# WGLab/ContextSV

Measured on AMD Instinct MI355X. Metric: long reads scanned/s (whole-genome step: scan + depth + cluster + merge + CN + split passes), synthetic 30x ONT WGS, higher is better.
Workload: dtype u32

## Files before the change

### contextsv_amd/csrc/kernels/scan.hip

```cpp
#include <type_traits>

#include "../common.hpp"
#include "../devutil.hpp"

namespace csv {

constexpr int SCAN_THREADS = 256;
constexpr int SCAN_WAVES = SCAN_THREADS / WAVE;
constexpr uint32_t SIG_BUF = 512;
constexpr int RING_D = 4;
constexpr int SCAN_OCC = 6;
constexpr int CHUNK_WORDS = 4 * WAVE;

struct Chunk {
    uint32_t w[4];
};

__device__ __forceinline__ void glds16(const uint32_t *gbase, uint32_t lane_byte_off, uint32_t lds_dst)
{
    unsigned keep;
    asm volatile("s_mov_b32 %0, m0\n\ts_mov_b32 m0, %3\n\ts_nop 0\n\tglobal_load_lds_dwordx4 %1, %2\n\ts_mov_b32 m0, %0"
                 : "=&s"(keep) : "v"(lane_byte_off), "s"(gbase), "s"(lds_dst) : "memory");
}
__device__ __forceinline__ uint32_t lds_addr(const void *p) { return (uint32_t)(uintptr_t)(__attribute__((address_space(3))) const void *)p; }

__device__ __forceinline__ void ring_issue(uint32_t *slot, const uint32_t *__restrict__ cigar, uint64_t base, int lane, uint64_t n_cigar, int vec_ok)
{
    const uint64_t idx = base + (uint64_t)lane * 4;
    if (vec_ok && base + CHUNK_WORDS <= n_cigar) {
        glds16(cigar + base, (uint32_t)lane * 16u, (uint32_t)__builtin_amdgcn_readfirstlane((int)lds_addr(slot)));
    } else {
#pragma unroll
        for (int k = 0; k < 4; k++) slot[lane * 4 + k] = (idx + k < n_cigar) ? cigar[idx + k] : (uint32_t)OP_P;
    }
}

__device__ __forceinline__ void ring_wait_steady()
{
    static_assert(RING_D >= 2 && RING_D <= 8, "add the immediate for RING_D - 1");
    if (RING_D == 8) asm volatile("s_waitcnt vmcnt(7)" ::: "memory");
    if (RING_D == 7) asm volatile("s_waitcnt vmcnt(6)" ::: "memory");
    if (RING_D == 6) asm volatile("s_waitcnt vmcnt(5)" ::: "memory");
    if (RING_D == 5) asm volatile("s_waitcnt vmcnt(4)" ::: "memory");
    if (RING_D == 4) asm volatile("s_waitcnt vmcnt(3)" ::: "memory");
    if (RING_D == 3) asm volatile("s_waitcnt vmcnt(2)" ::: "memory");
    if (RING_D == 2) asm volatile("s_waitcnt vmcnt(1)" ::: "memory");
}
__device__ __forceinline__ void ring_wait_all() { asm volatile("s_waitcnt vmcnt(0)" ::: "memory"); }

__device__ __forceinline__ uint64_t wave_lower_bound(const uint64_t *__restrict__ cigar_off, uint64_t n, uint64_t target, int lane)
{
    uint64_t lo = 0, hi = n;
    while (hi - lo > 0) {
        const uint64_t span = hi - lo;
        const uint64_t step = (span + 63) / 64;
        const uint64_t probe = lo + (uint64_t)lane * step;
        const bool ge = probe >= hi || cigar_off[probe] >= target;
        const uint64_t m = __ballot(ge);
        const int first_ge = m ? __ffsll((long long)m) - 1 : 64;
        const uint64_t new_hi = first_ge < 64 ? min(lo + (uint64_t)first_ge * step, hi) : hi;
        const uint64_t new_lo = first_ge > 0 ? lo + (uint64_t)(first_ge - 1) * step + 1 : lo;
        if (first_ge == 0) return lo;
        lo = new_lo; hi = new_hi;
        if (step == 1) return hi;
    }
    return lo;
}

__device__ __forceinline__ uint32_t bcast32(uint32_t v, uint32_t i) { return (uint32_t)__builtin_amdgcn_readlane((int)v, (int)i); }
__device__ __forceinline__ uint64_t bcast64(uint64_t v, uint32_t i)
{
    return ((uint64_t)bcast32((uint32_t)(v >> 32), i) << 32) | bcast32((uint32_t)v, i);
}
__global__ __launch_bounds__(SCAN_THREADS, SCAN_OCC) void cigar_scan_kernel(
    uint64_t n_reads, uint64_t n_cigar, const int32_t *__restrict__ pos, const uint16_t *__restrict__ flag,
    const uint8_t *__restrict__ mapq, const uint64_t *__restrict__ cigar_off, const uint32_t *__restrict__ cigar,
    int vec_ok, uint32_t depth_len, uint32_t start_limit, uint32_t min_oplen, uint32_t min_mapq, int emit,
    csv_sig *__restrict__ sig_out, uint64_t sig_cap, int32_t *__restrict__ ref_end, int32_t *__restrict__ q_start,
    int32_t *__restrict__ q_end, uint32_t *__restrict__ ckpt, ScanCounters *__restrict__ cnt,
    unsigned long long *__restrict__ tile_range, uint32_t n_tiles, uint32_t *__restrict__ bucket_hist, int hist_type_pos, int hist_shift,
    const uint64_t *__restrict__ split)
{
    __shared__ csv_sig buf[SIG_BUF];
    __shared__ alignas(16) uint32_t ring[SCAN_WAVES][RING_D][CHUNK_WORDS];
    __shared__ uint32_t buf_n, blk_n_del, blk_overflow;
    __shared__ unsigned long long blk_gbase;

    const int lane = lane_id();
    const int wave = (int)uniform32(threadIdx.x >> 6);
    if (threadIdx.x == 0) { buf_n = 0; blk_n_del = 0; blk_overflow = 0; }

    uint32_t my_n_del = 0, my_overflow = 0, my_bucket_max = 0;

    const uint64_t n_waves = (uint64_t)gridDim.x * SCAN_WAVES;
    const uint64_t wave_gid = (uint64_t)blockIdx.x * SCAN_WAVES + wave;
    const uint64_t share = (n_cigar + n_waves - 1) / n_waves;
    __shared__ uint64_t split_s[SCAN_WAVES + 1];
    __shared__ uint64_t split_w[SCAN_WAVES + 1];
    if (split) {
        if (threadIdx.x <= SCAN_WAVES) {
            const uint64_t g = (uint64_t)blockIdx.x * SCAN_WAVES + threadIdx.x;
            split_s[threadIdx.x] = split[2 * g]; split_w[threadIdx.x] = split[2 * g + 1];
        }
    } else {
        const uint64_t b = wave_lower_bound(cigar_off, n_reads, wave_gid * share, lane);
        if (lane == 0) split_s[wave] = b;
        if (wave == SCAN_WAVES - 1) {
            const uint64_t e = (wave_gid + 1 >= n_waves) ? n_reads : wave_lower_bound(cigar_off, n_reads, (wave_gid + 1) * share, lane);
            if (lane == 0) split_s[SCAN_WAVES] = e;
        }
    }
    __syncthreads();
    const uint64_t r_begin = uniform64(split_s[wave]);
    const uint64_t r_end = uniform64(split_s[wave + 1]);

    const uint64_t w_begin = split ? uniform64(split_w[wave]) : uniform64(r_begin < r_end ? cigar_off[r_begin] : 0);
    const uint64_t w_end = split ? uniform64(split_w[wave + 1]) : uniform64(r_begin < r_end ? cigar_off[r_end] : 0);
    const uint64_t ring_base = w_begin & ~(uint64_t)(CHUNK_WORDS - 1);
    const uint32_t ring_total = r_begin < r_end ? (uint32_t)((w_end - ring_base + CHUNK_WORDS - 1) / CHUNK_WORDS) : 0u;
    uint32_t ring_ready = 0;
    for (uint32_t a = 0; a < (uint32_t)(RING_D - 1) && a < ring_total; a++)
        ring_issue(ring[wave][a], cigar, ring_base + (uint64_t)a * CHUNK_WORDS, lane, n_cigar, vec_ok);

    for (uint64_t rb = r_begin; rb < r_end; rb += WAVE) {
    const uint64_t nb_reads = min((uint64_t)WAVE, r_end - rb);
    uint64_t l_c0 = 0; uint32_t l_p0 = 0, l_flmq = 0, l_uns = 0;
    if ((uint64_t)lane < nb_reads) {
        const uint64_t rr = rb + lane;
        l_c0 = cigar_off[rr];
        const int32_t p = pos[rr];
        l_p0 = (uint32_t)p; l_flmq = (uint32_t)flag[rr] | ((uint32_t)mapq[rr] << 16);
        l_uns = (rr > 0 && p < pos[rr - 1]) ? 1u : 0u;
    }
    const uint64_t batch_end_word = uniform64(cigar_off[rb + nb_reads]);
    if (__ballot(l_uns != 0) && lane == 0) cnt->unsorted = 1u;
    for (uint32_t ri = 0; ri < (uint32_t)nb_reads; ri++) {
        const uint64_t r = rb + ri;
        const bool have_next = ri + 1 < (uint32_t)nb_reads;
        const uint64_t c0 = bcast64(l_c0, ri);
        const uint64_t c1 = have_next ? bcast64(l_c0, ri + 1) : batch_end_word;
        const uint32_t p0 = bcast32(l_p0, ri);
        const uint32_t flmq = bcast32(l_flmq, ri);
        const uint32_t fl = flmq & 0xffffu, mq = flmq >> 16;
        const bool emit_ok = emit && !(fl & (F_SECONDARY | F_UNMAP | F_DUP | F_QCFAIL | F_SUPP)) && mq >= min_mapq;

        uint32_t ref_carry = 0;
        uint32_t acc_q = 0;
        uint32_t acc_skip = 0;
        bool had_skip = false;
        int32_t  qs = -1;

        const uint32_t n_words = (uint32_t)(c1 - c0);
        const uint32_t head = (uint32_t)c0 & (uint32_t)(CHUNK_WORDS - 1);
        const uint32_t n_chunks = n_words ? (head + n_words + CHUNK_WORDS - 1) / CHUNK_WORDS : 0u;
        const uint32_t j0 = (uint32_t)((c0 - head - ring_base) / CHUNK_WORDS);
        uint32_t *__restrict__ const ck_read = ckpt + ((c0 - head) >> CKPT_SHIFT);
        int32_t rel = lane * 4 - (int32_t)head;
        for (uint32_t t = 0; t < n_chunks; t++, rel += CHUNK_WORDS) {
            const uint32_t j = j0 + t;
            if (j == ring_ready) {
                const uint32_t ahead = j + (RING_D - 1);
                if (ahead < ring_total) {
                    ring_issue(ring[wave][ahead % RING_D], cigar, ring_base + (uint64_t)ahead * CHUNK_WORDS, lane, n_cigar, vec_ok);
                    ring_wait_steady();
                } else {
                    ring_wait_all();
                }
                ring_ready = j + 1;
            }
            Chunk cur;
            {
                const uint4 v = *reinterpret_cast<const uint4 *>(&ring[wave][j % RING_D][lane * 4]);
                cur.w[0] = v.x; cur.w[1] = v.y; cur.w[2] = v.z; cur.w[3] = v.w;
            }

            const bool edge = (t == 0 && head != 0) || (t + 1) * CHUNK_WORDS - head > n_words;
            if (edge) {
#pragma unroll
                for (int k = 0; k < 4; k++) if (!((uint32_t)(rel + k) < n_words)) cur.w[k] = (uint32_t)OP_P;
            }
            uint32_t len[4], op[4], rl[4], ql[4];
            uint32_t lane_ref = 0, lane_q = 0, trig = 0, qst = 0;
#pragma unroll
            for (int k = 0; k < 4; k++) {
                op[k] = cur.w[k] & 15u;
                len[k] = cur.w[k] >> 4;
                rl[k] = len[k] & (uint32_t)__builtin_amdgcn_sbfe((int)(REF_OPS | (REF_OPS << 16)), cur.w[k], 1u);
                ql[k] = len[k] & (uint32_t)__builtin_amdgcn_sbfe((int)(QRY_OPS | (QRY_OPS << 16)), cur.w[k], 1u);
                lane_ref += rl[k];
                lane_q += ql[k];
                trig |= rl[k] ^ ql[k];
            }
            const bool big = trig >= min_oplen;
            if (qs < 0) {
#pragma unroll
                for (int k = 0; k < 4; k++) qst |= (QST_OPS >> op[k]) & 1u;
            }
            const uint32_t incl_ref = wave_incl_sum_dpp(lane_ref);
            {
                static_assert(CKPT_WORDS == 64, "one checkpoint per DPP row of 16 lanes x 4 words");
                uint32_t *__restrict__ ck = ck_read + t * (CHUNK_WORDS / CKPT_WORDS);
                const bool inside = (edge || t == 0) ? (rel > 0 && (uint32_t)rel < n_words) : true;
                if ((lane & 15) == 0 && inside) ck[lane >> 4] = ref_carry + (incl_ref - lane_ref);
            }
            const bool any_big = emit_ok && __ballot(big) != 0;
            const bool need_q = (qs < 0) || any_big;
            if (need_q) {
                const uint32_t q_carry = t ? wave_total_dpp(acc_q) : 0u;
                const uint32_t incl_q = wave_incl_sum_dpp(lane_q);
                const uint32_t rp = p0 + ref_carry + (incl_ref - lane_ref);
                const uint32_t qp = q_carry + (incl_q - lane_q);

                if (qs < 0) {
                    const uint64_t m = __ballot(qst != 0);
                    if (m) {
                        bool found = false;
                        uint32_t q_at = 0, acc = qp;
#pragma unroll
                        for (int k = 0; k < 4; k++) {
                            if (!found && ((QST_OPS >> op[k]) & 1u)) { found = true; q_at = acc; }
                            acc += ql[k];
                        }
                        qs = (int32_t)bcast32(q_at, (uint32_t)(__ffsll((long long)m) - 1));
                    }
                }

                if (any_big) {
                    uint32_t cand = 0, skipped = 0, lane_skip = 0;
                    {
                        uint32_t rpk = rp;
#pragma unroll
                        for (int k = 0; k < 4; k++) {
                            if (len[k] >= min_oplen) {
                                if (op[k] == OP_I || op[k] == OP_D) cand |= 1u << k;
                                else if (op[k] == OP_S) {
                                    if ((uint32_t)(rpk + 1u) >= depth_len) { skipped |= 1u << k; lane_skip += len[k]; }
                                    else cand |= 1u << k;
                                }
                            }
                            rpk += rl[k];
                        }
                    }
                    uint32_t skip_before = had_skip ? wave_total_dpp(acc_skip) : 0u;
                    if (__ballot(skipped != 0)) {
                        skip_before += wave_incl_sum_dpp(lane_skip) - lane_skip;
                        acc_skip += lane_skip;
                        had_skip = true;
                    }
                    if (__ballot(cand != 0)) {
                        uint32_t rpk = rp, qpk = qp, skk = skip_before;
#pragma unroll
                        for (int k = 0; k < 4; k++) {
                            if ((cand >> k) & 1u) {
                                csv_sig sg;
                                sg.start = rpk + 1u;
                                sg.end = sg.start + len[k] - 1u;
                                sg.read = (uint32_t)r;
                                const uint32_t kind = (op[k] == OP_I) ? CSV_KIND_INS : (op[k] == OP_D ? CSV_KIND_DEL : CSV_KIND_CLIP);
                                sg.qpos_kind = ((qpk - skk) << 2) | kind;
                                const uint32_t slot = atomicAdd(&buf_n, 1u);
                                if (slot < SIG_BUF) buf[slot] = sg;
                                else {
                                    const unsigned long long g = atomicAdd(&cnt->n_sig, 1ull);
                                    if (g < sig_cap) sig_out[g] = sg;
                                    if (bucket_hist) my_bucket_max = max(my_bucket_max, atomicAdd(&bucket_hist[bk_bucket(sg, hist_type_pos, hist_shift)], 1u) + 1u);
                                }
                                my_n_del += (kind == CSV_KIND_DEL);
                                my_overflow |= (sg.start >= start_limit);
                            }
                            if ((skipped >> k) & 1u) skk += len[k];
                            rpk += rl[k];
                            qpk += ql[k];
                        }
                    }
                }
            }
            acc_q += lane_q;
            ref_carry += (uint32_t)__builtin_amdgcn_readlane((int)incl_ref, 63);
        }

        if (tile_range && ref_carry != 0 && !(fl & (F_UNMAP | F_SECONDARY | F_QCFAIL | F_DUP))) {
            const uint32_t first = p0 + 1u, last = first + ref_carry - 1u;
            const uint32_t t0 = first >> DEPTH_TILE_SHIFT;
            if (t0 < n_tiles && last >= first) {
                const uint32_t t1 = min(last >> DEPTH_TILE_SHIFT, n_tiles - 1u);
                for (uint32_t t = t0 + (uint32_t)lane; t <= t1; t += WAVE) {
                    atomicMax(&tile_range[2 * (uint64_t)t], ~(unsigned long long)r);
                    atomicMax(&tile_range[2 * (uint64_t)t + 1], (unsigned long long)r + 1ull);
                }
            }
        }

        const uint32_t q_total = wave_total_dpp(acc_q);
        if (lane == 0) {
            uint32_t rlen = (fl & F_UNMAP) ? 0u : ref_carry;
            if (rlen == 0) rlen = 1;
            ref_end[r] = (int32_t)(p0 + rlen);
            q_start[r] = qs < 0 ? 0 : qs;
            q_end[r] = (int32_t)q_total;
        }
    }
    }
    ring_wait_all();

    if (!emit) return;
    my_n_del = wave_sum(my_n_del);
    const bool wave_overflow = __ballot(my_overflow != 0) != 0;
    if (lane == 0) {
        if (my_n_del) atomicAdd(&blk_n_del, my_n_del);
        if (wave_overflow) atomicOr(&blk_overflow, 1u);
    }
    __syncthreads();
    const uint32_t nb = min(buf_n, SIG_BUF);
    if (threadIdx.x == 0) {
        blk_gbase = nb ? atomicAdd(&cnt->n_sig, (unsigned long long)nb) : 0ull;
        if (blk_n_del) atomicAdd(&cnt->n_del, (unsigned long long)blk_n_del);
        if (blk_overflow) cnt->max_start = 0xffffffffu;
    }
    __syncthreads();
    const unsigned long long g = blk_gbase;
    for (uint32_t i = threadIdx.x; i < nb; i += SCAN_THREADS) {
        const csv_sig sg = buf[i];
        if (g + i < sig_cap) sig_out[g + i] = sg;
        if (bucket_hist) my_bucket_max = max(my_bucket_max, atomicAdd(&bucket_hist[bk_bucket(sg, hist_type_pos, hist_shift)], 1u) + 1u);
    }
    if (bucket_hist) {
        my_bucket_max = wave_max(my_bucket_max);
        if (lane == 0 && my_bucket_max > BK_LOCAL_MAX) atomicMax(&cnt->max_len, my_bucket_max);
    }
}

constexpr int RS_THREADS = 256;
constexpr int RS_WAVES = RS_THREADS / WAVE;
constexpr int rs_occ(int gl) { return gl == 8 ? 5 : 7; }
constexpr uint32_t TR_SLOTS = 64;
constexpr uint32_t RS_MIN_READS = 32;

template <int GL, bool PADDED>
__global__ __launch_bounds__(RS_THREADS, rs_occ(GL)) void cigar_scan_rows_kernel(
    uint64_t n_reads, uint64_t n_cigar, const int32_t *__restrict__ pos, const uint16_t *__restrict__ flag,
    const uint8_t *__restrict__ mapq, const uint64_t *__restrict__ cigar_off, const uint32_t *__restrict__ cigar,
    uint32_t depth_len, uint32_t start_limit, uint32_t min_oplen, uint32_t min_mapq, int emit,
    csv_sig *__restrict__ sig_out, uint64_t sig_cap, int32_t *__restrict__ ref_end, int32_t *__restrict__ q_start,
    int32_t *__restrict__ q_end, uint32_t *__restrict__ ckpt, ScanCounters *__restrict__ cnt,
    unsigned long long *__restrict__ tile_range, uint32_t n_tiles, uint32_t *__restrict__ bucket_hist, int hist_type_pos, int hist_shift,
    const uint64_t *__restrict__ split)
{
    constexpr int WPL = WAVE / GL;
    constexpr int NG = WAVE / GL;
    __shared__ csv_sig buf[SIG_BUF];
    __shared__ alignas(16) uint4 meta[RS_WAVES][WAVE];
    __shared__ uint32_t tr_first[TR_SLOTS], tr_last[TR_SLOTS];
    __shared__ uint32_t buf_n, blk_n_del, blk_overflow, tr_base;
    __shared__ unsigned long long blk_gbase;
    __shared__ uint64_t split_s[RS_WAVES + 1];

    const int lane = lane_id();
    const int wave = (int)uniform32(threadIdx.x >> 6);
    const uint32_t sub = (uint32_t)lane & (uint32_t)(GL - 1);
    const uint32_t grp = (uint32_t)lane / (uint32_t)GL;
    const uint32_t upper = (lane & 8) ? 0xffffffffu : 0u;
    if (threadIdx.x == 0) { buf_n = 0; blk_n_del = 0; blk_overflow = 0; }
    if (threadIdx.x < TR_SLOTS) { tr_first[threadIdx.x] = 0; tr_last[threadIdx.x] = 0; }

    const uint64_t n_waves = (uint64_t)gridDim.x * RS_WAVES;
    const uint64_t wave_gid = (uint64_t)blockIdx.x * RS_WAVES + wave;
    const uint64_t share = (n_cigar + n_waves - 1) / n_waves;
    if (split) {
        if (threadIdx.x <= RS_WAVES) split_s[threadIdx.x] = split[2 * ((uint64_t)blockIdx.x * RS_WAVES + threadIdx.x)];
    } else {
        const uint64_t b = wave_lower_bound(cigar_off, n_reads, wave_gid * share, lane);
        if (lane == 0) split_s[wave] = b;
        if (wave == RS_WAVES - 1) {
            const uint64_t e = (wave_gid + 1 >= n_waves) ? n_reads : wave_lower_bound(cigar_off, n_reads, (wave_gid + 1) * share, lane);
            if (lane == 0) split_s[RS_WAVES] = e;
        }
    }
    __syncthreads();
    if (threadIdx.x == 0) {
        const uint64_t r0 = split_s[0];
        tr_base = (tile_range && r0 < n_reads) ? (((uint32_t)pos[r0] + 1u) >> DEPTH_TILE_SHIFT) : 0u;
    }
    __syncthreads();
    const uint64_t r_begin = uniform64(split_s[wave]);
    const uint64_t r_end = uniform64(split_s[wave + 1]);
    const uint32_t tbase = tr_base;

    uint32_t my_n_del = 0, my_overflow = 0, my_bucket_max = 0;

    auto loadw = [&](uint32_t g, uint32_t (&w)[WPL]) {
        if (PADDED) {
#pragma unroll
            for (int q = 0; q < WPL; q += 4) {
                const uint4 x = *reinterpret_cast<const uint4 *>(cigar + g + q);
                w[q] = x.x; w[q + 1] = x.y; w[q + 2] = x.z; w[q + 3] = x.w;
            }
        } else {
#pragma unroll
            for (int k = 0; k < WPL; k++) w[k] = ((uint64_t)g + k < n_cigar) ? cigar[g + k] : (uint32_t)OP_P;
        }
    };

    for (uint64_t rb = r_begin; rb < r_end; rb += WAVE) {
        const uint32_t nb = (uint32_t)min((uint64_t)WAVE, r_end - rb);
        uint32_t l_p0 = 0, l_fl = 0;
        {
            uint4 m = make_uint4(0u, 0u, 0u, 0u);
            uint32_t l_uns = 0;
            if ((uint32_t)lane < nb) {
                const uint64_t rr = rb + lane;
                const uint64_t c0 = cigar_off[rr], c1 = cigar_off[rr + 1];
                const int32_t p = pos[rr];
                m = make_uint4((uint32_t)c0, (uint32_t)(c1 - c0), (uint32_t)p, (uint32_t)flag[rr] | ((uint32_t)mapq[rr] << 16));
                l_p0 = m.z; l_fl = m.w & 0xffffu;
                l_uns = (rr > 0 && p < pos[rr - 1]) ? 1u : 0u;
            }
            if (__ballot(l_uns != 0) && lane == 0) cnt->unsorted = 1u;
            __builtin_amdgcn_fence(__ATOMIC_RELEASE, "wavefront");
            meta[wave][lane] = m;
            __builtin_amdgcn_fence(__ATOMIC_RELEASE, "wavefront");
            __builtin_amdgcn_wave_barrier();
            __builtin_amdgcn_fence(__ATOMIC_ACQUIRE, "wavefront");
        }
        uint32_t slot = grp;
        bool act = slot < nb;
        uint4 cm = meta[wave][act ? slot : 0u];
        uint32_t v = 0;
        uint32_t ref_carry = 0, q_carry = 0, skip_carry = 0;
        int32_t qs = -1;
        uint32_t w[WPL];
        loadw(act ? (cm.x & ~3u) + sub * WPL : 0u, w);
        while (__ballot(act)) {
            const uint32_t c0 = cm.x, nw = act ? cm.y : 0u, p0 = cm.z, fl = cm.w & 0xffffu, mq = cm.w >> 16;
            const uint32_t a = c0 & ~3u;
            const uint32_t n_win = max(1u, (c0 - a + nw + 63u) >> 6);
            const bool last = v + 1 >= n_win;
            const uint32_t nslot = last ? slot + NG : slot;
            const bool nact = act && nslot < nb;
            uint4 nm = cm;
            if (last) nm = meta[wave][nact ? nslot : 0u];
            const uint32_t nv = last ? 0u : v + 1u;
            uint32_t wn[WPL];
            loadw(nact ? (nm.x & ~3u) + nv * 64u + sub * WPL : 0u, wn);

            const uint32_t g = a + v * 64u + sub * WPL;
            const uint32_t t = g - c0;
            const bool emit_ok = emit && act && !(fl & (F_SECONDARY | F_UNMAP | F_DUP | F_QCFAIL | F_SUPP)) && mq >= min_mapq;
            uint32_t lane_ref = 0, lane_q = 0, trig = 0;
#pragma unroll
            for (int k = 0; k < WPL; k++) {
                if (!((uint32_t)(t + k) < nw)) w[k] = (uint32_t)OP_P;
                const uint32_t len = w[k] >> 4;
                const uint32_t rl = len & (uint32_t)__builtin_amdgcn_sbfe((int)(REF_OPS | (REF_OPS << 16)), w[k], 1u);
                const uint32_t ql = len & (uint32_t)__builtin_amdgcn_sbfe((int)(QRY_OPS | (QRY_OPS << 16)), w[k], 1u);
                lane_ref += rl; lane_q += ql;
                trig |= rl ^ ql;
            }
            const uint32_t incl_ref = grp_incl_sum<GL>(lane_ref, upper);
            const uint32_t incl_q = grp_incl_sum<GL>(lane_q, upper);
            const uint32_t tot_ref = grp_last<GL>(incl_ref), tot_q = grp_last<GL>(incl_q);
            const uint32_t ro = ref_carry + (incl_ref - lane_ref);
            const uint32_t qp = q_carry + (incl_q - lane_q);
            {
                if ((g & (uint32_t)(CKPT_WORDS - 1)) == 0 && t - 1u < nw - 1u && nw) ckpt[g >> CKPT_SHIFT] = ro;
                if (WPL == 8 && ((g + 4u) & (uint32_t)(CKPT_WORDS - 1)) == 0 && t + 3u < nw - 1u && nw) {
                    uint32_t x = ro;
#pragma unroll
                    for (int k = 0; k < 4; k++) x += (w[k] >> 4) & (uint32_t)__builtin_amdgcn_sbfe((int)(REF_OPS | (REF_OPS << 16)), w[k], 1u);
                    ckpt[(g + 4u) >> CKPT_SHIFT] = x;
                }
            }
            if (__ballot(qs < 0 && act)) {
                uint32_t q_at = 0xffffffffu, acc = qp;
                bool found = false;
#pragma unroll
                for (int k = 0; k < WPL; k++) {
                    const uint32_t op = w[k] & 15u;
                    if (!found && ((QST_OPS >> op) & 1u)) { found = true; q_at = acc; }
                    acc += (w[k] >> 4) & (uint32_t)__builtin_amdgcn_sbfe((int)(QRY_OPS | (QRY_OPS << 16)), w[k], 1u);
                }
                const uint32_t first = grp_min<GL>(q_at);
                if (qs < 0 && first != 0xffffffffu) qs = (int32_t)first;
            }
            uint32_t skip_tot = 0;
            if (__ballot(emit_ok && trig >= min_oplen)) {
                constexpr uint32_t ISD_OPS = (1u << OP_I) | (1u << OP_S) | (1u << OP_D);
                uint32_t cand = 0, skipped = 0;
                if (emit_ok) {
#pragma unroll
                    for (int k = 0; k < WPL; k++)
                        if ((w[k] >> 4) >= min_oplen && __builtin_amdgcn_sbfe((int)(ISD_OPS | (ISD_OPS << 16)), w[k], 1u)) cand |= 1u << k;
                }
                const bool may_skip = ((p0 | ref_carry | tot_ref) >= 0x20000000u) || (p0 + ref_carry + tot_ref + 1u >= depth_len);
                uint32_t skip_before = skip_carry;
                if (__ballot(cand != 0 && may_skip)) {
                    uint32_t lane_skip = 0, rpk = p0 + ro;
#pragma unroll
                    for (int k = 0; k < WPL; k++) {
                        const uint32_t len = w[k] >> 4, op = w[k] & 15u;
                        if (((cand >> k) & 1u) && op == OP_S && (uint32_t)(rpk + 1u) >= depth_len) { skipped |= 1u << k; lane_skip += len; }
                        rpk += len & (uint32_t)__builtin_amdgcn_sbfe((int)(REF_OPS | (REF_OPS << 16)), w[k], 1u);
                    }
                    cand &= ~skipped;
                    const uint32_t is = grp_incl_sum<GL>(lane_skip, upper);
                    skip_before += is - lane_skip;
                    skip_tot = grp_last<GL>(is);
                }
                if (cand) {
                    uint32_t rpk = p0 + ro, qpk = qp, skk = skip_before;
#pragma unroll
                    for (int k = 0; k < WPL; k++) {
                        const uint32_t len = w[k] >> 4, op = w[k] & 15u;
                        if ((cand >> k) & 1u) {
                            csv_sig sg;
                            sg.start = rpk + 1u;
                            sg.end = sg.start + len - 1u;
                            sg.read = (uint32_t)rb + slot;
                            const uint32_t kind = (op == OP_I) ? CSV_KIND_INS : (op == OP_D ? CSV_KIND_DEL : CSV_KIND_CLIP);
                            sg.qpos_kind = ((qpk - skk) << 2) | kind;
                            const uint32_t sl = atomicAdd(&buf_n, 1u);
                            if (sl < SIG_BUF) buf[sl] = sg;
                            else {
                                const unsigned long long gi = atomicAdd(&cnt->n_sig, 1ull);
                                if (gi < sig_cap) sig_out[gi] = sg;
                                if (bucket_hist) my_bucket_max = max(my_bucket_max, atomicAdd(&bucket_hist[bk_bucket(sg, hist_type_pos, hist_shift)], 1u) + 1u);
                            }
                            my_n_del += (kind == CSV_KIND_DEL);
                            my_overflow |= (sg.start >= start_limit);
                        }
                        if ((skipped >> k) & 1u) skk += len;
                        rpk += len & (uint32_t)__builtin_amdgcn_sbfe((int)(REF_OPS | (REF_OPS << 16)), w[k], 1u);
                        qpk += len & (uint32_t)__builtin_amdgcn_sbfe((int)(QRY_OPS | (QRY_OPS << 16)), w[k], 1u);
                    }
                }
            }
            const uint32_t ref_total = ref_carry + tot_ref, q_total = q_carry + tot_q;
            if (last && act && sub == 0) meta[wave][slot] = make_uint4(ref_total, (uint32_t)qs, q_total, 0u);
            if (last) { ref_carry = 0; q_carry = 0; skip_carry = 0; qs = -1; v = 0; slot = nslot; cm = nm; act = nact; }
            else { ref_carry = ref_total; q_carry = q_total; skip_carry += skip_tot; v = nv; }
#pragma unroll
            for (int k = 0; k < WPL; k++) w[k] = wn[k];
        }
        __builtin_amdgcn_fence(__ATOMIC_RELEASE, "wavefront");
        __builtin_amdgcn_wave_barrier();
        __builtin_amdgcn_fence(__ATOMIC_ACQUIRE, "wavefront");
        {
            const bool mine = (uint32_t)lane < nb;
            const uint4 res = meta[wave][lane];
            const uint64_t rr = rb + lane;
            if (mine) {
                uint32_t rlen = (l_fl & F_UNMAP) ? 0u : res.x;
                if (rlen == 0) rlen = 1;
                ref_end[rr] = (int32_t)(l_p0 + rlen);
                q_start[rr] = (int32_t)res.y < 0 ? 0 : (int32_t)res.y;
                q_end[rr] = (int32_t)res.z;
            }
            uint32_t t0 = 1, t1 = 0;
            if (mine && tile_range && res.x != 0 && !(l_fl & (F_UNMAP | F_SECONDARY | F_QCFAIL | F_DUP))) {
                const uint32_t first = l_p0 + 1u, lastp = first + res.x - 1u;
                if ((first >> DEPTH_TILE_SHIFT) < n_tiles && lastp >= first) { t0 = first >> DEPTH_TILE_SHIFT; t1 = min(lastp >> DEPTH_TILE_SHIFT, n_tiles - 1u); }
            }
            auto mark = [&](uint32_t tt, uint32_t rd) {
                const uint32_t sl = tt - tbase;
                if (sl < TR_SLOTS) {
                    atomicMax(&tr_first[sl], ~rd);
                    atomicMax(&tr_last[sl], rd + 1u);
                } else {
                    atomicMax(&tile_range[2 * (uint64_t)tt], ~(unsigned long long)rd);
                    atomicMax(&tile_range[2 * (uint64_t)tt + 1], (unsigned long long)rd + 1ull);
                }
            };
            const bool wide = t1 >= t0 && t1 - t0 >= 8u;
            if (t1 >= t0 && !wide) for (uint32_t tt = t0; tt <= t1; tt++) mark(tt, (uint32_t)rr);
            for (uint64_t mw = __ballot(wide); mw; mw &= mw - 1) {
                const uint32_t src = (uint32_t)__builtin_ctzll(mw);
                const uint32_t a0 = bcast32(t0, src), a1 = bcast32(t1, src), rd = (uint32_t)rb + src;
                for (uint32_t tt = a0 + (uint32_t)lane; tt <= a1; tt += WAVE) mark(tt, rd);
            }
        }
        __builtin_amdgcn_fence(__ATOMIC_RELEASE, "wavefront");
        __builtin_amdgcn_wave_barrier();
    }
// ... 363 lines not shown
```

Baseline: 321.0 million.

## Add a specialized steady-state CIGAR chunk loop with hand-scheduled DPP scan

Splits the per-read chunk loop into a head chunk, a steady-state middle loop and a generic tail. The middle loop always issues the direct-to-LDS DMA, skips edge masking and the ring-ready checks, and interleaves the query-length decode with DPP prefix-sum steps behind sched_barriers. The query-start search is also computed in the head chunk with ballots rather than a separate scan. The aim is to cut per-chunk control overhead and DPP latency stalls in the dominant scan loop, at the cost of more code, an m0 clobber that relies on the compiler, and a more fragile ring-index bookkeeping.

Result: no change. 322.3 million (median of 3 runs) (+0.4%).

```diff
diff --git a/contextsv_amd/csrc/kernels/scan.hip b/contextsv_amd/csrc/kernels/scan.hip
--- a/contextsv_amd/csrc/kernels/scan.hip
+++ b/contextsv_amd/csrc/kernels/scan.hip
@@ -22,6 +22,14 @@
     asm volatile("s_mov_b32 %0, m0\n\ts_mov_b32 m0, %3\n\ts_nop 0\n\tglobal_load_lds_dwordx4 %1, %2\n\ts_mov_b32 m0, %0"
                  : "=&s"(keep) : "v"(lane_byte_off), "s"(gbase), "s"(lds_dst) : "memory");
 }
+#pragma clang diagnostic push
+#pragma clang diagnostic ignored "-Winline-asm"
+__device__ __forceinline__ void glds16_m0(const uint32_t *gbase, uint32_t lane_byte_off, uint32_t lds_dst)
+{
+    asm volatile("s_mov_b32 m0, %2\n\ts_nop 0\n\tglobal_load_lds_dwordx4 %0, %1"
+                 : : "v"(lane_byte_off), "s"(gbase), "s"(lds_dst) : "memory", "m0");
+}
+#pragma clang diagnostic pop
 __device__ __forceinline__ uint32_t lds_addr(const void *p) { return (uint32_t)(uintptr_t)(__attribute__((address_space(3))) const void *)p; }
 
 __device__ __forceinline__ void ring_issue(uint32_t *slot, const uint32_t *__restrict__ cigar, uint64_t base, int lane, uint64_t n_cigar, int vec_ok)
@@ -121,6 +129,9 @@
     uint32_t ring_ready = 0;
     for (uint32_t a = 0; a < (uint32_t)(RING_D - 1) && a < ring_total; a++)
         ring_issue(ring[wave][a], cigar, ring_base + (uint64_t)a * CHUNK_WORDS, lane, n_cigar, vec_ok);
+    const uint32_t dma_chunks = vec_ok ? (uint32_t)min((uint64_t)ring_total, (n_cigar - ring_base) / CHUNK_WORDS) : 0u;
+    const uint32_t ring_lds = uniform32(lds_addr(&ring[wave][0][0]));
+    const uint32_t lane16 = (uint32_t)lane * 16u;
 
     for (uint64_t rb = r_begin; rb < r_end; rb += WAVE) {
     const uint64_t nb_reads = min((uint64_t)WAVE, r_end - rb);
@@ -155,8 +166,83 @@
         const uint32_t n_chunks = n_words ? (head + n_words + CHUNK_WORDS - 1) / CHUNK_WORDS : 0u;
         const uint32_t j0 = (uint32_t)((c0 - head - ring_base) / CHUNK_WORDS);
         uint32_t *__restrict__ const ck_read = ckpt + ((c0 - head) >> CKPT_SHIFT);
-        int32_t rel = lane * 4 - (int32_t)head;
-        for (uint32_t t = 0; t < n_chunks; t++, rel += CHUNK_WORDS) {
+
+        auto decode = [&](const Chunk &cur, uint32_t (&rl)[4], uint32_t (&ql)[4], uint32_t &lane_ref, uint32_t &lane_q, uint32_t &trig) __attribute__((always_inline)) {
+            lane_ref = 0; lane_q = 0; trig = 0;
+#pragma unroll
+            for (int k = 0; k < 4; k++) {
+                const uint32_t len = cur.w[k] >> 4;
+                rl[k] = len & (uint32_t)__builtin_amdgcn_sbfe((int)(REF_OPS | (REF_OPS << 16)), cur.w[k], 1u);
+                ql[k] = len & (uint32_t)__builtin_amdgcn_sbfe((int)(QRY_OPS | (QRY_OPS << 16)), cur.w[k], 1u);
+                lane_ref += rl[k];
+                lane_q += ql[k];
+                trig |= rl[k] ^ ql[k];
+            }
+        };
+
+        auto signatures = [&](const Chunk &cur, uint32_t rp, uint32_t qp) __attribute__((always_inline)) {
+            uint32_t op[4], len[4], rl[4], ql[4];
+#pragma unroll
+            for (int k = 0; k < 4; k++) {
+                uint32_t w = cur.w[k];
+                asm volatile("" : "+v"(w));
+                op[k] = w & 15u;
+                len[k] = w >> 4;
+                rl[k] = len[k] & (uint32_t)__builtin_amdgcn_sbfe((int)(REF_OPS | (REF_OPS << 16)), w, 1u);
+                ql[k] = len[k] & (uint32_t)__builtin_amdgcn_sbfe((int)(QRY_OPS | (QRY_OPS << 16)), w, 1u);
+            }
+            uint32_t cand = 0, skipped = 0, lane_skip = 0;
+            {
+                uint32_t rpk = rp;
+#pragma unroll
+                for (int k = 0; k < 4; k++) {
+                    if (len[k] >= min_oplen) {
+                        if (op[k] == OP_I || op[k] == OP_D) cand |= 1u << k;
+                        else if (op[k] == OP_S) {
+                            if ((uint32_t)(rpk + 1u) >= depth_len) { skipped |= 1u << k; lane_skip += len[k]; }
+                            else cand |= 1u << k;
+                        }
+                    }
+                    rpk += rl[k];
+                }
+            }
+            uint32_t skip_before = had_skip ? wave_total_dpp(acc_skip) : 0u;
+            if (__ballot(skipped != 0)) {
+                skip_before += wave_incl_sum_dpp(lane_skip) - lane_skip;
+                acc_skip += lane_skip;
+                had_skip = true;
+            }
+            if (__ballot(cand != 0)) {
+                uint32_t rpk = rp, qpk = qp, skk = skip_before;
+#pragma unroll
+                for (int k = 0; k < 4; k++) {
+                    if ((cand >> k) & 1u) {
+                        csv_sig sg;
+                        sg.start = rpk + 1u;
+                        sg.end = sg.start + len[k] - 1u;
+                        sg.read = (uint32_t)r;
+                        const uint32_t kind = (op[k] == OP_I) ? CSV_KIND_INS : (op[k] == OP_D ? CSV_KIND_DEL : CSV_KIND_CLIP);
+                        sg.qpos_kind = ((qpk - skk) << 2) | kind;
+                        const uint32_t slot = atomicAdd(&buf_n, 1u);
+                        if (slot < SIG_BUF) buf[slot] = sg;
+                        else {
+                            const unsigned long long g = atomicAdd(&cnt->n_sig, 1ull);
+                            if (g < sig_cap) sig_out[g] = sg;
+                            if (bucket_hist) my_bucket_max = max(my_bucket_max, atomicAdd(&bucket_hist[bk_bucket(sg, hist_type_pos, hist_shift)], 1u) + 1u);
+                        }
+                        my_n_del += (kind == CSV_KIND_DEL);
+                        my_overflow |= (sg.start >= start_limit);
+                    }
+                    if ((skipped >> k) & 1u) skk += len[k];
+                    rpk += rl[k];
+                    qpk += ql[k];
+                }
+            }
+        };
+
+        auto visit = [&](auto is_head, const uint32_t t) __attribute__((always_inline)) {
+            constexpr bool HEAD = decltype(is_head)::value;
+            const int32_t rel = lane * 4 + (int32_t)(t * CHUNK_WORDS) - (int32_t)head;
             const uint32_t j = j0 + t;
             if (j == ring_ready) {
                 const uint32_t ahead = j + (RING_D - 1);
@@ -174,110 +260,120 @@
                 cur.w[0] = v.x; cur.w[1] = v.y; cur.w[2] = v.z; cur.w[3] = v.w;
             }
 
-            const bool edge = (t == 0 && head != 0) || (t + 1) * CHUNK_WORDS - head > n_words;
+            const bool edge = (HEAD && head != 0) || (t + 1) * CHUNK_WORDS - head > n_words;
             if (edge) {
 #pragma unroll
                 for (int k = 0; k < 4; k++) if (!((uint32_t)(rel + k) < n_words)) cur.w[k] = (uint32_t)OP_P;
             }
-            uint32_t len[4], op[4], rl[4], ql[4];
-            uint32_t lane_ref = 0, lane_q = 0, trig = 0, qst = 0;
-#pragma unroll
-            for (int k = 0; k < 4; k++) {
-                op[k] = cur.w[k] & 15u;
-                len[k] = cur.w[k] >> 4;
-                rl[k] = len[k] & (uint32_t)__builtin_amdgcn_sbfe((int)(REF_OPS | (REF_OPS << 16)), cur.w[k], 1u);
-                ql[k] = len[k] & (uint32_t)__builtin_amdgcn_sbfe((int)(QRY_OPS | (QRY_OPS << 16)), cur.w[k], 1u);
-                lane_ref += rl[k];
-                lane_q += ql[k];
-                trig |= rl[k] ^ ql[k];
-            }
+            uint32_t rl[4], ql[4], lane_ref, lane_q, trig;
+            decode(cur, rl, ql, lane_ref, lane_q, trig);
             const bool big = trig >= min_oplen;
+            uint64_t qst_lanes = 0;
+            uint32_t pre_q = 0;
             if (qs < 0) {
-#pragma unroll
-                for (int k = 0; k < 4; k++) qst |= (QST_OPS >> op[k]) & 1u;
+                uint32_t h[4];
+#pragma unroll
+                for (int k = 0; k < 4; k++) h[k] = (uint32_t)__builtin_amdgcn_sbfe((int)(QST_OPS | (QST_OPS << 16)), cur.w[k], 1u);
+                uint32_t seen = h[0];
+                pre_q = ql[0] & ~seen;
+                seen |= h[1]; pre_q += ql[1] & ~seen;
+                seen |= h[2]; pre_q += ql[2] & ~seen;
+                seen |= h[3];
+                qst_lanes = __ballot(seen != 0);
+                if (HEAD && qst_lanes) {
+                    const uint32_t F = (uint32_t)__builtin_ctzll(qst_lanes);
+                    if ((__ballot(lane_q != 0) & ((1ull << F) - 1ull)) == 0) { qs = (int32_t)bcast32(pre_q, F); qst_lanes = 0; }
+                }
             }
             const uint32_t incl_ref = wave_incl_sum_dpp(lane_ref);
             {
                 static_assert(CKPT_WORDS == 64, "one checkpoint per DPP row of 16 lanes x 4 words");
                 uint32_t *__restrict__ ck = ck_read + t * (CHUNK_WORDS / CKPT_WORDS);
-                const bool inside = (edge || t == 0) ? (rel > 0 && (uint32_t)rel < n_words) : true;
+                const bool inside = (edge || HEAD) ? (rel > 0 && (uint32_t)rel < n_words) : true;
                 if ((lane & 15) == 0 && inside) ck[lane >> 4] = ref_carry + (incl_ref - lane_ref);
             }
             const bool any_big = emit_ok && __ballot(big) != 0;
-            const bool need_q = (qs < 0) || any_big;
-            if (need_q) {
-                const uint32_t q_carry = t ? wave_total_dpp(acc_q) : 0u;
+            if (qst_lanes != 0 || any_big) {
+                const uint32_t q_carry = HEAD ? 0u : wave_total_dpp(acc_q);
                 const uint32_t incl_q = wave_incl_sum_dpp(lane_q);
-                const uint32_t rp = p0 + ref_carry + (incl_ref - lane_ref);
                 const uint32_t qp = q_carry + (incl_q - lane_q);
-
-                if (qs < 0) {
-                    const uint64_t m = __ballot(qst != 0);
-                    if (m) {
-                        bool found = false;
-                        uint32_t q_at = 0, acc = qp;
-#pragma unroll
-                        for (int k = 0; k < 4; k++) {
-                            if (!found && ((QST_OPS >> op[k]) & 1u)) { found = true; q_at = acc; }
-                            acc += ql[k];
-                        }
-                        qs = (int32_t)bcast32(q_at, (uint32_t)(__ffsll((long long)m) - 1));
-                    }
-                }
-
-                if (any_big) {
-                    uint32_t cand = 0, skipped = 0, lane_skip = 0;
-                    {
-                        uint32_t rpk = rp;
-#pragma unroll
-                        for (int k = 0; k < 4; k++) {
-                            if (len[k] >= min_oplen) {
-                                if (op[k] == OP_I || op[k] == OP_D) cand |= 1u << k;
-                                else if (op[k] == OP_S) {
-                                    if ((uint32_t)(rpk + 1u) >= depth_len) { skipped |= 1u << k; lane_skip += len[k]; }
-                                    else cand |= 1u << k;
-                                }
-                            }
-                            rpk += rl[k];
-                        }
-                    }
-                    uint32_t skip_before = had_skip ? wave_total_dpp(acc_skip) : 0u;
-                    if (__ballot(skipped != 0)) {
-                        skip_before += wave_incl_sum_dpp(lane_skip) - lane_skip;
-                        acc_skip += lane_skip;
-                        had_skip = true;
-                    }
-                    if (__ballot(cand != 0)) {
-                        uint32_t rpk = rp, qpk = qp, skk = skip_before;
-#pragma unroll
-                        for (int k = 0; k < 4; k++) {
-                            if ((cand >> k) & 1u) {
-                                csv_sig sg;
-                                sg.start = rpk + 1u;
-                                sg.end = sg.start + len[k] - 1u;
-                                sg.read = (uint32_t)r;
-                                const uint32_t kind = (op[k] == OP_I) ? CSV_KIND_INS : (op[k] == OP_D ? CSV_KIND_DEL : CSV_KIND_CLIP);
-                                sg.qpos_kind = ((qpk - skk) << 2) | kind;
-                                const uint32_t slot = atomicAdd(&buf_n, 1u);
-                                if (slot < SIG_BUF) buf[slot] = sg;
-                                else {
-                                    const unsigned long long g = atomicAdd(&cnt->n_sig, 1ull);
-                                    if (g < sig_cap) sig_out[g] = sg;
-                                    if (bucket_hist) my_bucket_max = max(my_bucket_max, atomicAdd(&bucket_hist[bk_bucket(sg, hist_type_pos, hist_shift)], 1u) + 1u);
-                                }
-                                my_n_del += (kind == CSV_KIND_DEL);
-                                my_overflow |= (sg.start >= start_limit);
-                            }
-                            if ((skipped >> k) & 1u) skk += len[k];
-                            rpk += rl[k];
-                            qpk += ql[k];
-                        }
-                    }
-                }
+                if (qst_lanes) qs = (int32_t)bcast32(qp + pre_q, (uint32_t)__builtin_ctzll(qst_lanes));
+                if (any_big) signatures(cur, p0 + ref_carry + (incl_ref - lane_ref), qp);
             }
             acc_q += lane_q;
             ref_carry += (uint32_t)__builtin_amdgcn_readlane((int)incl_ref, 63);
-        }
+        };
+
+        uint32_t t = 0;
+        if (n_chunks) { visit(std::true_type{}, 0u); t = 1; }
+        if (qs >= 0 && n_chunks > 2) {
+            const uint32_t reach = j0 + (uint32_t)RING_D;
+            const uint32_t t_end = dma_chunks > reach ? min(n_chunks - 1u, dma_chunks - reach + 1u) : 1u;
+            if (t_end > 1u) {
+                uint32_t slot = ((j0 + (uint32_t)RING_D) % RING_D) * (uint32_t)(CHUNK_WORDS * 4);
+                const uint32_t *gp = cigar + ring_base + (uint64_t)reach * CHUNK_WORDS;
+                uint32_t *__restrict__ ck = ck_read + (CHUNK_WORDS / CKPT_WORDS) + (lane >> 4);
+                const bool ck_lane = (lane & 15) == 0;
+                for (; t < t_end; t++) {
+                    glds16_m0(gp, lane16, ring_lds + slot);
+                    ring_wait_steady();
+                    gp += CHUNK_WORDS;
+                    slot = (slot + (uint32_t)(CHUNK_WORDS * 4)) % (uint32_t)(RING_D * CHUNK_WORDS * 4);
+                    Chunk cur;
+                    {
+                        const uint4 v = *reinterpret_cast<const uint4 *>(reinterpret_cast<const char *>(&ring[wave][0][0]) + slot + lane16);
+                        cur.w[0] = v.x; cur.w[1] = v.y; cur.w[2] = v.z; cur.w[3] = v.w;
+                    }
+                    uint32_t rl[4], ql[4], lane_ref = 0, lane_q, trig = 0;
+                    const auto qlen = [&](int k) { return (cur.w[k] >> 4) & (uint32_t)__builtin_amdgcn_sbfe((int)(QRY_OPS | (QRY_OPS << 16)), cur.w[k], 1u); };
+#pragma unroll
+                    for (int k = 0; k < 4; k++) {
+                        rl[k] = (cur.w[k] >> 4) & (uint32_t)__builtin_amdgcn_sbfe((int)(REF_OPS | (REF_OPS << 16)), cur.w[k], 1u);
+                        lane_ref += rl[k];
+                    }
+                    uint32_t incl_ref = lane_ref;
+                    __builtin_amdgcn_sched_barrier(0);
+                    ql[0] = qlen(0); asm volatile("" : "+v"(ql[0]));
+                    __builtin_amdgcn_sched_barrier(0);
+                    incl_ref += dpp_u32<0x111, 0xf>(0u, incl_ref);
+                    __builtin_amdgcn_sched_barrier(0);
+                    ql[1] = qlen(1); asm volatile("" : "+v"(ql[1]));
+                    __builtin_amdgcn_sched_barrier(0);
+                    incl_ref += dpp_u32<0x112, 0xf>(0u, incl_ref);
+                    __builtin_amdgcn_sched_barrier(0);
+                    ql[2] = qlen(2); asm volatile("" : "+v"(ql[2]));
+                    __builtin_amdgcn_sched_barrier(0);
+                    incl_ref += dpp_u32<0x114, 0xf>(0u, incl_ref);
+                    __builtin_amdgcn_sched_barrier(0);
+                    ql[3] = qlen(3); asm volatile("" : "+v"(ql[3]));
+                    __builtin_amdgcn_sched_barrier(0);
+                    incl_ref += dpp_u32<0x118, 0xf>(0u, incl_ref);
+                    __builtin_amdgcn_sched_barrier(0);
+                    lane_q = ql[0] + ql[1] + ql[2] + ql[3]; asm volatile("" : "+v"(lane_q));
+                    __builtin_amdgcn_sched_barrier(0);
+                    incl_ref += dpp_u32<0x142, 0xa>(0u, incl_ref);
+                    __builtin_amdgcn_sched_barrier(0);
+                    uint32_t ck_base = ref_carry - lane_ref; asm volatile("" : "+v"(ck_base));
+                    uint32_t *__restrict__ const ck_here = ck;
+                    ck += CHUNK_WORDS / CKPT_WORDS;
+                    __builtin_amdgcn_sched_barrier(0);
+                    incl_ref += dpp_u32<0x143, 0xc>(0u, incl_ref);
+                    __builtin_amdgcn_sched_barrier(0);
+                    if (ck_lane) *ck_here = ck_base + incl_ref;
+#pragma unroll
+                    for (int k = 0; k < 4; k++) trig |= rl[k] ^ ql[k];
+                    if (emit_ok && __ballot(trig >= min_oplen) != 0) {
+                        const uint32_t q_carry = wave_total_dpp(acc_q);
+                        const uint32_t incl_q = wave_incl_sum_dpp(lane_q);
+                        signatures(cur, p0 + ref_carry + (incl_ref - lane_ref), q_carry + (incl_q - lane_q));
+                    }
+                    acc_q += lane_q;
+                    ref_carry += (uint32_t)__builtin_amdgcn_readlane((int)incl_ref, 63);
+                }
+                ring_ready = j0 + t_end;
+            }
+        }
+        for (; t < n_chunks; t++) visit(std::false_type{}, t);
 
         if (tile_range && ref_carry != 0 && !(fl & (F_UNMAP | F_SECONDARY | F_QCFAIL | F_DUP))) {
             const uint32_t first = p0 + 1u, last = first + ref_carry - 1u;
```
